# zhengjingsen/LidarDetection

Measured on AMD Instinct MI355X. Metric: frames/sec (fwd+NMS) PointPillar-KITTI, higher is better.
Workload: dtype f32; 1 GPU; PointPillar-KITTI bs=16 per GPU, fp32, eval BN folded: HIP voxelize + PFN; dense 2D backbone = first layer from the pillars (sparse implicit GEMM), stride-1 3x3 layers as Winograd F(4x4,3x3) on the fp32 MFMA, strided deblocks as one fused MFMA GEMM (all this repo's HIP), the two stride-2 3x3 layers MIOpen, stride-1 deblock + 1x1 heads hipBLASLt; exact HIP top-k + decode + batched rotated NMS; clou; replicas=1

## Files before the change

include/lidar_hip.h:

```cpp
#ifndef LIDAR_HIP_H
#define LIDAR_HIP_H

#include <stddef.h>
#include <stdint.h>

#ifdef __cplusplus
extern "C" {
#endif

#define LIDAR_OK 0
#define LIDAR_ERR_ARG (-1)
#define LIDAR_ERR_LAUNCH (-2)
#define LIDAR_ERR_WORKSPACE (-3)
#define LIDAR_ERR_UNSUPPORTED (-4)

size_t lidar_voxelize_workspace_bytes(int batch, int n_max, int max_voxels);
int lidar_voxelize_workspace_init(void *ws, size_t ws_bytes, int batch, int n_max, int max_voxels, void *stream);
int lidar_voxelize(const float *points, const int *point_offsets, int batch, int n_max, int num_features,
                   const float *range6, const float *voxel_size3, const int *grid3, int max_points,
                   int max_voxels, int compact, int algo, float *voxels, int *coords, int *num_points,
                   int *voxel_offsets, void *ws, size_t ws_bytes, void *stream);
int lidar_voxelize_hostoff(const float *points, const int *point_offsets, const int *host_offsets, int batch, int n_max,
                           int num_features, const float *range6, const float *voxel_size3, const int *grid3, int max_points,
                           int max_voxels, int compact, int algo, float *voxels, int *coords, int *num_points,
// ... 7 lines not shown
                                    void *stream);
int lidar_voxelize_error_flag(void *ws, size_t ws_bytes, int batch, int n_max, int max_voxels);

size_t lidar_voxelize_cpu_scratch_bytes(int n);
int lidar_voxelize_cpu(const float *points, int n, int num_features, const float *range6, const float *voxel_size3,
                       const int *grid3, int max_points, int max_voxels, float *voxels, int *coords_zyx, int *num_points,
                       void *scratch, size_t scratch_bytes);

int lidar_pillar_vfe(const float *voxels, const void *num_points, const void *coords, int num_voxels,
                     const int *num_voxels_dev, int max_points, int num_features, const float *weight,
                     const float *scale, const float *shift, int cout, const float *voxel_size3,
                     const float *range6, int with_distance, int coords_are_float, int num_are_float,
                     float *out, void *stream);

int lidar_mean_vfe(const float *voxels, const void *num_points, int num_voxels, int max_points,
                   int num_features, int num_are_float, float *out, void *stream);

int lidar_pillar_scatter_update(const float *pillar_features, const void *coords, int coords_are_float, int num_voxels,
                                const int *num_voxels_dev, int channels, int batch, int nx, int ny, float *canvas,
                                int *prev_cells, int *prev_count, void *stream);
size_t lidar_pillar_conv_table_workspace_bytes(int batch, int nx, int ny);
int lidar_pillar_conv_table(const void *coords, int coords_are_float, int num_voxels, const int *num_voxels_dev, int batch, int nx,
                            int ny, int k, int stride, int pad, int *nbr, void *ws, size_t ws_bytes, void *stream);
size_t lidar_pillar_scatter_workspace_bytes(int batch, int nx, int ny);
int lidar_pillar_scatter(const float *pillar_features, const void *coords, int coords_are_float, int num_voxels,
                         const int *num_voxels_dev, int channels, int batch, int nx, int ny, int channels_last,
                         float *canvas, void *ws, size_t ws_bytes, void *stream);

size_t lidar_pfn_train_workspace_bytes(int num_voxels, int num_features, int cout, int with_distance);
int lidar_pfn_train_forward(const float *voxels, const void *num_points, const void *coords, int num_voxels, const int *num_voxels_dev,
                            int max_points, int num_features, const float *weight, const float *gamma, const float *beta, int cout,
                            float eps, const float *voxel_size3, const float *range6, int with_distance, int coords_are_float,
                            int num_are_float, float *out, float *zsel, unsigned char *slot, double *stats, float *scale_shift,
                            float *batch_stats, void *ws, size_t ws_bytes, void *stream);
int lidar_pfn_train_backward(const float *voxels, const void *num_points, const void *coords, int num_voxels, const int *num_voxels_dev,
                             int max_points, int num_features, const float *weight, const float *gamma, int cout,
                             const float *voxel_size3, const float *range6, int with_distance, int coords_are_float, int num_are_float,
                             const float *grad_out, const float *zsel, const unsigned char *slot, const double *stats,
                             const float *scale_shift, float *d_weight, float *d_gamma, float *d_beta, void *ws, size_t ws_bytes,
                             void *stream);
int lidar_pillar_scatter_backward(const float *grad_canvas, const void *coords, int coords_are_float, int num_voxels,
                                  const int *num_voxels_dev, int channels, int batch, int nx, int ny, int channels_last,
                                  float *grad_features, void *stream);

size_t lidar_bn_relu_train_workspace_bytes(long long rows, int channels);
int lidar_bn_relu_train_forward(int nseg, void *const *x, const int *x_ld, const int *x_off, const int *seg_C, long long rows,
// ... 113 lines not shown
int lidar_spconv_grid_table(const int *out_indices, int n_out, int batch, int D, int H, int W, int kD, int kH, int kW, int sD, int sH, int sW,
                            int pD, int pH, int pW, const int *grid_in, int limit, int *nbr, void *stream);
int lidar_spconv_grid_table_t(const int *indices, int n, int batch, int D, int H, int W, int kD, int kH, int kW, int sD, int sH, int sW, int pD,
                              int pH, int pW, const int *grid_out, int limit, int *nbr_t, void *stream);
int lidar_spconv_grid_pad_rows(int *out_indices, const int *num_dev, int cap, void *stream);
int lidar_spconv_transpose_table(const int *nbr, int n_out, int K, int n_in, int *nbr_t, void *stream);
size_t lidar_spconv_grid_outputs_workspace_bytes(int n, int K);
int lidar_spconv_grid_outputs(const int *indices, int n, int batch, int D, int H, int W, int kD, int kH, int kW, int sD, int sH, int sW, int pD,
                              int pH, int pW, int *grid_out, int *out_indices, int *num_out, void *ws, size_t ws_bytes,
                              void *stream);
int lidar_spconv_implicit_gemm(const float *in_features, const int *nbr, int n_out, int K, int Cin, int Cout,
                               const float *weight, const float *bias, float *out_features, void *stream);
int lidar_spconv_implicit_gemm_fused(const float *in_features, const int *nbr, int n_out, int K, int Cin, int Cout,
                                     const float *weight, const float *bias, const float *residual, int relu,
                                     float *out_features, void *stream);
int lidar_spconv_row_masks(const int *nbr, int n_out, int K, int *masks, void *stream);
size_t lidar_spconv_mask_group_workspace_bytes(int n_out);
int lidar_spconv_mask_group_init(void *ws, size_t ws_bytes, void *stream);
int lidar_spconv_mask_group(const int *nbr, int n_out, int K, int *masks, int *order, void *ws, size_t ws_bytes, void *stream);
int lidar_spconv_sorted_gemm_supported(int K, int Cin, int Cout);
int lidar_spconv_implicit_gemm_sorted(const float *in_features, const int *nbr, const int *row_mask, const int *order,
                                      int n_out, int K, int Cin, int Cout, const float *weight, const float *bias,
                                      const float *residual, int relu, float *out_features, void *stream);
size_t lidar_spconv_packed_floats(int K, int Cin, int Cout);
int lidar_spconv_pack_weights(const float *weight, int K, int Cin, int Cout, float *packed, void *stream);
int lidar_spconv_implicit_gemm_sorted_packed(const float *in_features, const int *nbr, const int *row_mask, const int *order,
                                             int n_out, int K, int Cin, int Cout, const float *packed, const float *bias,
                                             const float *residual, int relu, float *out_features, void *stream);
int lidar_spconv_wgrad(const float *in_features, const float *grad_out, const int *nbr, int n_out, int K, int Cin, int Cout,
                       float *grad_weight, void *stream);
int lidar_spconv_wgrad_mfma_supported(int K, int Cin, int Cout);
size_t lidar_spconv_wgrad_workspace_bytes(int n_out, int K, int Cin, int Cout);
int lidar_spconv_wgrad_mfma(const float *in_features, const float *grad_out, const int *nbr, const int *order, int n_out, int K,
                            int Cin, int Cout, float *grad_weight, void *ws, size_t ws_bytes, void *stream);
size_t lidar_sparse_to_dense_workspace_bytes(int batch, int D, int H, int W);
int lidar_sparse_to_dense(const float *features, const int *indices, int n, int channels, int batch, int D, int H, int W,
                          float *out, void *ws, size_t ws_bytes, void *stream);

int lidar_bias_act_nhwc(const float *in, const float *bias, long long n_pix, int C, int relu, float *out, int out_C,
                        int out_off, void *stream);
int lidar_bias_act_upsample_nhwc(const float *in, const float *bias, int batch, int h, int w, int s, int C, int relu,
                                 float *out, int out_C, int out_off, void *stream);
int lidar_dense_gemm_bias_act(const float *A, long long M, int K, const float *W, int N, const float *bias, int relu,
                              float *D, int ldd, void *ws, size_t ws_bytes, void *stream);
int lidar_dense_gemm_export_choices(int *out7, int cap);
int lidar_dense_gemm_import_choices(const int *in7, int n);
// ... 198 lines not shown
```

lidardetection_amd/_lib.py:

```python
import ctypes as C
import os

_HERE = os.path.dirname(os.path.abspath(__file__))
SO_PATH = os.environ.get("LIDAR_HIP_SO") or os.path.join(_HERE, "csrc", "liblidar_hip.so")

vp, i32, f32, sz = C.c_void_p, C.c_int, C.c_float, C.c_size_t

SIGNATURES = {
    "lidar_voxelize_workspace_bytes": (sz, [i32, i32, i32]),
    "lidar_voxelize_workspace_init": (i32, [vp, sz, i32, i32, i32, vp]),
    "lidar_voxelize": (i32, [vp, vp, i32, i32, i32, vp, vp, vp, i32, i32, i32, i32, vp, vp, vp, vp, vp, sz, vp]),
    "lidar_voxelize_hostoff": (i32, [vp, vp, vp, i32, i32, i32, vp, vp, vp, i32, i32, i32, i32, vp, vp, vp, vp, vp, sz, vp]),
    "lidar_voxelize_error_flag": (i32, [vp, sz, i32, i32, i32]),
    "lidar_timer_create": (vp, []),
    "lidar_timer_destroy": (None, [vp]),
    "lidar_voxelize_time_next": (None, [vp]),
    "lidar_timer_elapsed_ms": (C.c_float, [vp]),
    "lidar_timer_parts_ms": (i32, [vp, vp]),
    "lidar_voxelize_set_error_mirror": (i32, [vp, sz, i32, i32, i32, vp, vp]),
    "lidar_pillar_vfe": (i32, [vp, vp, vp, i32, vp, i32, i32, vp, vp, vp, i32, vp, vp, i32, i32, i32, vp, vp]),
    "lidar_mean_vfe": (i32, [vp, vp, i32, i32, i32, i32, vp, vp]),
    "lidar_pillar_scatter_workspace_bytes": (sz, [i32, i32, i32]),
    "lidar_pillar_scatter": (i32, [vp, vp, i32, i32, vp, i32, i32, i32, i32, i32, vp, vp, sz, vp]),
    "lidar_pillar_scatter_update": (i32, [vp, vp, i32, i32, vp, i32, i32, i32, i32, vp, vp, vp, vp]),
    "lidar_pillar_conv_table_workspace_bytes": (sz, [i32, i32, i32]),
    "lidar_pillar_conv_table": (i32, [vp, i32, i32, vp, i32, i32, i32, i32, i32, i32, vp, vp, sz, vp]),
    "lidar_pfn_train_workspace_bytes": (sz, [i32, i32, i32, i32]),
    "lidar_pfn_train_forward": (i32, [vp, vp, vp, i32, vp, i32, i32, vp, vp, vp, i32, f32, vp, vp, i32, i32, i32, vp, vp, vp, vp, vp,
                                      vp, vp, sz, vp]),
    "lidar_pfn_train_backward": (i32, [vp, vp, vp, i32, vp, i32, i32, vp, vp, i32, vp, vp, i32, i32, i32, vp, vp, vp, vp, vp, vp, vp,
                                       vp, vp, sz, vp]),
    "lidar_pillar_scatter_backward": (i32, [vp, vp, i32, i32, vp, i32, i32, i32, i32, i32, vp, vp]),
    "lidar_bn_relu_train_workspace_bytes": (sz, [C.c_longlong, i32]),
    "lidar_bn_relu_train_forward": (i32, [i32, vp, vp, vp, vp, C.c_longlong, vp, vp, f32, vp, i32, i32, vp, vp, vp, vp, sz, vp]),
    "lidar_bn_relu_train_backward": (i32, [i32, vp, vp, vp, vp, C.c_longlong, vp, i32, i32, vp, vp, vp, vp, vp, vp, vp, sz, vp]),
    "lidar_bn_add_relu_train_forward": (i32, [vp, i32, vp, i32, i32, C.c_longlong, vp, vp, f32, vp, i32, vp, vp, vp, vp, sz, vp]),
    "lidar_bn_add_relu_train_backward": (i32, [vp, i32, vp, i32, i32, C.c_longlong, vp, i32, vp, vp, vp, vp, vp, i32, vp, vp, vp, sz, vp]),
    "lidar_iou_workspace_bytes": (sz, [i32, i32]),
    "lidar_boxes_pairwise_bev": (i32, [vp, i32, vp, i32, i32, vp, vp, sz, vp]),
    "lidar_nms_workspace_bytes": (sz, [i32, i32]),
    "lidar_nms_batch": (i32, [vp, vp, i32, i32, f32, i32, vp, vp, vp, sz, vp]),
    "lidar_nms_batch_limited": (i32, [vp, vp, i32, i32, f32, i32, i32, vp, vp, vp, sz, vp]),
    "lidar_nms_mask_ptr": (vp, [vp, i32, i32]),
    "lidar_ball_query_stack": (i32, [i32, i32, f32, i32, vp, vp, vp, vp, vp, vp]),
    "lidar_ball_query_stack2": (i32, [i32, i32, f32, i32, f32, i32, vp, vp, vp, vp, vp, vp, vp]),
    "lidar_ball_query_grid_workspace_bytes": (sz, [i32, i32]),
    "lidar_ball_query_stack_grid": (i32, [i32, i32, i32, f32, i32, f32, i32, vp, vp, vp, vp, vp, vp, vp, sz, vp]),
    "lidar_group_points_stack": (i32, [i32, i32, i32, i32, vp, vp, vp, vp, vp, vp]),
    "lidar_group_rows_stack": (i32, [i32, i32, i32, i32, i32, i32, vp, vp, vp, vp, vp, vp, vp, vp]),
# ... 27 lines not shown
    "lidar_roipoint_pool3d_forward": (i32, [i32, i32, i32, i32, i32, vp, vp, vp, vp, vp, vp]),
    "lidar_spconv_hash_capacity": (sz, [i32]),
    "lidar_spconv_build_hash": (i32, [vp, i32, i32, i32, i32, vp, sz, vp]),
    "lidar_spconv_subm_table": (i32, [vp, i32, i32, i32, i32, i32, i32, i32, vp, sz, vp, vp]),
    "lidar_spconv_conv_table_workspace_bytes": (sz, [i32, i32, i32, i32, i32, i32, i32]),
    "lidar_spconv_conv_outputs": (i32, [vp, i32, i32, i32, i32, i32, i32, i32, i32, i32, i32, i32, i32, i32, i32, vp, i32, vp, vp, sz, vp]),
    "lidar_spconv_conv_tables": (i32, [i32, i32, i32, i32, i32, i32, i32, i32, vp, vp, vp, sz, vp]),
    "lidar_spconv_grid_init": (i32, [vp, sz, vp]),
    "lidar_spconv_grid_rows": (i32, [vp, i32, vp, i32, i32, i32, i32, vp, i32, vp]),
    "lidar_spconv_grid_table": (i32, [vp, i32, i32, i32, i32, i32, i32, i32, i32, i32, i32, i32, i32, i32, i32, vp, i32, vp, vp]),
    "lidar_spconv_grid_table_t": (i32, [vp, i32, i32, i32, i32, i32, i32, i32, i32, i32, i32, i32, i32, i32, i32, vp, i32, vp, vp]),
    "lidar_spconv_grid_pad_rows": (i32, [vp, vp, i32, vp]),
    "lidar_spconv_transpose_table": (i32, [vp, i32, i32, i32, vp, vp]),
    "lidar_spconv_grid_outputs_workspace_bytes": (sz, [i32, i32]),
    "lidar_spconv_grid_outputs": (i32, [vp, i32, i32, i32, i32, i32, i32, i32, i32, i32, i32, i32, i32, i32, i32, vp, vp, vp, vp, sz, vp]),
    "lidar_spconv_implicit_gemm": (i32, [vp, vp, i32, i32, i32, i32, vp, vp, vp, vp]),
    "lidar_spconv_implicit_gemm_fused": (i32, [vp, vp, i32, i32, i32, i32, vp, vp, vp, i32, vp, vp]),
    "lidar_spconv_row_masks": (i32, [vp, i32, i32, vp, vp]),
    "lidar_spconv_mask_group_workspace_bytes": (sz, [i32]),
    "lidar_spconv_mask_group_init": (i32, [vp, sz, vp]),
    "lidar_spconv_mask_group": (i32, [vp, i32, i32, vp, vp, vp, sz, vp]),
    "lidar_spconv_sorted_gemm_supported": (i32, [i32, i32, i32]),
    "lidar_spconv_implicit_gemm_sorted": (i32, [vp, vp, vp, vp, i32, i32, i32, i32, vp, vp, vp, i32, vp, vp]),
    "lidar_spconv_packed_floats": (sz, [i32, i32, i32]),
    "lidar_spconv_pack_weights": (i32, [vp, i32, i32, i32, vp, vp]),
    "lidar_spconv_implicit_gemm_sorted_packed": (i32, [vp, vp, vp, vp, i32, i32, i32, i32, vp, vp, vp, i32, vp, vp]),
    "lidar_spconv_wgrad": (i32, [vp, vp, vp, i32, i32, i32, i32, vp, vp]),
    "lidar_spconv_wgrad_mfma_supported": (i32, [i32, i32, i32]),
    "lidar_spconv_wgrad_workspace_bytes": (sz, [i32, i32, i32, i32]),
    "lidar_spconv_wgrad_mfma": (i32, [vp, vp, vp, vp, i32, i32, i32, i32, vp, vp, sz, vp]),
    "lidar_sparse_to_dense_workspace_bytes": (sz, [i32, i32, i32, i32]),
    "lidar_sparse_to_dense": (i32, [vp, vp, i32, i32, i32, i32, i32, i32, vp, vp, sz, vp]),
    "lidar_sparse_to_bev_nhwc": (i32, [vp, vp, i32, i32, i32, i32, i32, i32, vp, vp, sz, vp]),
    "lidar_sparse_to_bev_nhwc_backward": (i32, [vp, i32, i32, vp, i32, i32, i32, i32, i32, i32, vp, vp]),
    "lidar_bias_act_nhwc": (i32, [vp, vp, C.c_longlong, i32, i32, vp, i32, i32, vp]),
    "lidar_bias_act_upsample_nhwc": (i32, [vp, vp, i32, i32, i32, i32, i32, i32, vp, i32, i32, vp]),
    "lidar_dense_gemm_bias_act": (i32, [vp, C.c_longlong, i32, vp, i32, vp, i32, vp, i32, vp, sz, vp]),
    "lidar_dense_gemm_export_choices": (i32, [vp, i32]),
    "lidar_dense_gemm_import_choices": (i32, [vp, i32]),
    "lidar_wino_packed_floats": (sz, [i32, i32]),
    "lidar_wino_supported": (i32, [i32, i32]),
    "lidar_wino_pack_weights": (i32, [vp, i32, i32, vp, vp]),
    "lidar_wino_conv3x3_nhwc": (i32, [vp, i32, i32, i32, i32, vp, vp, i32, i32, vp, i32, i32, vp]),
    "lidar_wino43_packed_floats": (sz, [i32, i32]),
    "lidar_wino43_supported": (i32, [i32, i32]),
    "lidar_wino43_pack_weights": (i32, [vp, i32, i32, vp, vp]),
# ... 183 lines not shown
```

lidardetection_amd/bev_backbone.py:

```python
import ctypes as C
import os
from typing import NamedTuple, Optional

import torch
import torch.nn as nn
import torch.nn.functional as F

from . import _lib, wino, workspace


def bias_act_(x, bias, relu=True, out=None, out_offset=0):
    _lib.require_cuda(bias)
    if not (x.is_cuda and x.dim() == 4 and x.is_contiguous(memory_format=torch.channels_last)):
        raise _lib.LidarHipError("bias_act_: expected a channels-last CUDA tensor")
    B, C, H, W = x.shape
    out, out_offset = (x, 0) if out is None else _lib.nhwc_out("bias_act_", B, (H, W), C, x.device, out, out_offset)
    _lib.check(_lib.lib().lidar_bias_act_nhwc(_lib.ptr(x), _lib.ptr(bias), B * H * W, C, int(bool(relu)), _lib.ptr(out),
                                              out.shape[1], int(out_offset), _lib.stream()), "lidar_bias_act_nhwc")
    return out


_LT_GEMM = [os.environ.get("LIDAR_BEV_LT_GEMM", "1") != "0"]
_SPLIT_MIN = [int(os.environ.get("LIDAR_BEV_SPLIT_MIN", "8"))]
_SPLIT = [int(os.environ.get("LIDAR_BEV_SPLIT", "2"))]
_WINO = [os.environ.get("LIDAR_BEV_WINO", "1") != "0"]
_DECONV = [os.environ.get("LIDAR_BEV_DECONV", "1") != "0"]
_SPARSE_FIRST = [os.environ.get("LIDAR_BEV_SPARSE_FIRST", "1") != "0"]


def _lt_gemm(a_ptr, M, K, w_kn, bias, relu, d_ptr, ldd, device):
    ws = workspace.get("dense_gemm", 32 << 20, device)
    st = _lib.lib().lidar_dense_gemm_bias_act(a_ptr, M, K, _lib.ptr(w_kn), w_kn.shape[1], _lib.ptr(bias), int(bool(relu)), d_ptr, ldd,
                                              _lib.ptr(ws), ws.numel(), _lib.stream())
    if st == -4:
        return False
    _lib.check(st, "lidar_dense_gemm_bias_act")
    return True


def _side_streams(device, n):
    from .spconv import conv as _sc, modules as _sm
    dev = torch.device(device)
    out = []
    for pool in (_sc._SIDE_STREAMS, _sm._RULEBOOK_STREAMS)[:n]:
        st = pool.get(dev)
        if st is None:
            st = pool[dev] = torch.cuda.Stream(dev, priority=-1)
        out.append(st)
    return out
# ... 198 lines not shown
        for h in heads:
            assert tuple(h.kernel_size) == (1, 1) and tuple(h.stride) == (1, 1)
        self.head_split = [h.weight.shape[0] for h in heads]
        if heads:
            self.head_wt = torch.cat([h.weight.detach().flatten(1) for h in heads], 0).t().contiguous()
            self.head_b = torch.cat([h.bias.detach() if h.bias is not None else h.weight.new_zeros(h.weight.shape[0])
                                     for h in heads], 0).contiguous()
        self._cats = {}
        self._streams = None
        self._first_sparse = None
        c0 = self.stages[0][0][0]
        w0, b0, st0, pad0 = c0.weight, c0.shift, c0.stride, c0.pad
        k0 = w0.shape[2]
        if (w0.is_cuda and w0.shape[2] == w0.shape[3] and st0[0] == st0[1] and pad0[0] == pad0[1] and k0 * k0 <= 31
                and c0.dilation == (1, 1) and c0.groups == 1 and c0.zero_pad is None):
            from .spconv import ops as _sops
            if _sops.sorted_gemm_supported(k0 * k0, w0.shape[1], w0.shape[0]):
                self._first_sparse = (w0.permute(2, 3, 1, 0).reshape(k0 * k0, w0.shape[1], w0.shape[0]).contiguous(), b0, k0, int(st0[0]), int(pad0[0]))

    def first_layer_from_pillars(self, pm):
        from . import pillar_ops
        from .spconv import ops as _sops
        w9, b0, k0, st0, pad0 = self._first_sparse
        nbr, OH, OW = pillar_ops.pillar_conv_table(pm.coords, pm.B, pm.nx, pm.ny, k0, st0, pad0, pm.num_voxels_dev)
        order = _sops.mask_order(nbr)
        out = _sops.indice_conv_fused(pm.features, nbr, w9, b0, None, True, order)
        return out.view(pm.B, OH, OW, w9.shape[2]).permute(0, 3, 1, 2)

    def sparse_first_ok(self):
        return self._first_sparse is not None and _SPARSE_FIRST[0]

    def features(self, canvas, slot=0, first_done=False):
        x, cat, off = canvas, None, 0
        for si, (convs, up) in enumerate(self.stages):
            for ci, cv in enumerate(convs):
                if first_done and si == 0 and ci == 0:
                    continue
                if cv.wino is not None and _WINO[0] and x.is_contiguous(memory_format=torch.channels_last):
                    x = wino.conv3x3_auto(x, cv.wino, cv.weight.shape[0], cv.shift, True)
                    continue
                if cv.zero_pad is not None:
                    x = F.pad(x, cv.zero_pad)
                x = _cl(F.conv2d(x, cv.weight, None, cv.stride, cv.pad, cv.dilation, cv.groups))
                bias_act_(x, cv.shift)
            B, _, h, w = x.shape
            y = None
# ... 69 lines not shown
```

lidardetection_amd/csrc/pillar.hip:

```cpp
#include "common.h"

struct PfnParams {
    float vx, vy, vz, xo, yo, zo;
    int P, C, cout, nfeat;
    int with_distance, coords_are_float, num_are_float;
};

__device__ __forceinline__ float pfn_sum32(float v) {
    v += __int_as_float(__builtin_amdgcn_update_dpp(0, __float_as_int(v), 0xB1, 0xf, 0xf, true));
    v += __int_as_float(__builtin_amdgcn_update_dpp(0, __float_as_int(v), 0x4E, 0xf, 0xf, true));
    v += __int_as_float(__builtin_amdgcn_update_dpp(0, __float_as_int(v), 0x141, 0xf, 0xf, true));
    v += __int_as_float(__builtin_amdgcn_update_dpp(0, __float_as_int(v), 0x140, 0xf, 0xf, true));
    return __int_as_float(__builtin_amdgcn_readlane(__float_as_int(v), 0)) + __int_as_float(__builtin_amdgcn_readlane(__float_as_int(v), 16));
}

template <int C, bool DIST>
__global__ __launch_bounds__(256) void pfn_kernel(const float *__restrict__ voxels, const void *__restrict__ num_points,
                                                  const void *__restrict__ coords, const float *__restrict__ weight ,
                                                  const float *__restrict__ scale, const float *__restrict__ shift,
                                                  const int *__restrict__ nvox_dev, int nvox_host, PfnParams p,
                                                  float *__restrict__ out ) {
    constexpr int NF = C + 6 + (DIST ? 1 : 0);
    const int l = lane_id();
    const int nv = nvox_dev ? min(*nvox_dev, nvox_host) : nvox_host;
// ... 426 lines not shown
}

LIDAR_EXPORT int lidar_pillar_conv_table(const void *coords, int coords_are_float, int num_voxels, const int *num_voxels_dev, int batch,
                                         int nx, int ny, int k, int stride, int pad, int *nbr, void *ws, size_t ws_bytes, void *stream) {
    if (!coords || !nbr || !ws || batch <= 0 || nx <= 0 || ny <= 0 || num_voxels < 0 || k <= 0 || k > 5 || stride <= 0 || pad < 0)
        return LIDAR_ERR_ARG;
    if (ws_bytes < lidar_pillar_conv_table_workspace_bytes(batch, nx, ny)) return LIDAR_ERR_WORKSPACE;
    const int OH = (ny + 2 * pad - k) / stride + 1, OW = (nx + 2 * pad - k) / stride + 1;
    if (OH <= 0 || OW <= 0) return LIDAR_ERR_ARG;
    const long long cells = (long long)batch * nx * ny, total = (long long)batch * OH * OW * k * k;
    if (cells > 0x7fffffffll || total > 0x7fffffffll * 256ll) return LIDAR_ERR_ARG;
    hipStream_t s = (hipStream_t)stream;
    int *map = (int *)ws;
    int fb = divup(cells, 256 * 4);
    if (fb > 2048) fb = 2048;
    hipLaunchKernelGGL(scatter_fill_kernel, dim3(fb), dim3(256), 0, s, map, cells);
    if (num_voxels > 0)
        hipLaunchKernelGGL(scatter_index_kernel, dim3(divup(num_voxels, 256)), dim3(256), 0, s, coords, coords_are_float, num_voxels,
                           num_voxels_dev, batch, nx, ny, ny, map);
    hipLaunchKernelGGL(pillar_conv_table_kernel, dim3((unsigned)divup(total, 256)), dim3(256), 0, s, map, batch, ny, nx, OH, OW, k, stride, pad, nbr);
    return lidar_check_launch("lidar_pillar_conv_table");
}

template <int CH>
__global__ __launch_bounds__(256) void canvas_clear_cells_kernel(const int *__restrict__ prev_cells, const int *__restrict__ prev_count,
                                                                 int cap, float *__restrict__ canvas) {
    constexpr int Q = CH / 4;
    const long long e = (long long)blockIdx.x * 256 + threadIdx.x;
    const int n = min(*prev_count, cap);
    const long long v = e / Q;
    if (v >= n) return;
    const int cell = prev_cells[v];
    if (cell >= 0) reinterpret_cast<float4 *>(canvas)[(long long)cell * Q + (e - v * Q)] = make_float4(0.f, 0.f, 0.f, 0.f);
}

template <int CH>
__global__ __launch_bounds__(256) void canvas_write_cells_kernel(const float *__restrict__ feat, const void *__restrict__ coords,
                                                                 int coords_are_float, int nvox_host, const int *__restrict__ nvox_dev,
                                                                 int B, int nx, int ny, float *__restrict__ canvas,
                                                                 int *__restrict__ prev_cells, int *__restrict__ prev_count) {
    constexpr int Q = CH / 4;
    const int nv = nvox_dev ? min(*nvox_dev, nvox_host) : nvox_host;
    const long long e = (long long)blockIdx.x * 256 + threadIdx.x;
    if (e == 0) *prev_count = nv;
    const long long v = e / Q;
    if (v >= nv) return;
// ... 110 lines not shown
```

lidardetection_amd/csrc/sparse_conv.hip:

```cpp
#include "common.h"
#ifndef SC_PROBE
#define SC_PROBE 0
#endif
#include <stdlib.h>

#define SC_EMPTY 0xFFFFFFFFFFFFFFFFull

struct ScGeom {
    int B, D, H, W;
    int oD, oH, oW;
    int kD, kH, kW, K;
    int sD, sH, sW, pD, pH, pW;
};

__device__ __forceinline__ unsigned long long sc_key(int b, int z, int y, int x, int D, int H, int W) {
    return (((unsigned long long)b * D + z) * H + y) * W + x;
}

__device__ __forceinline__ unsigned sc_hash(unsigned long long key, unsigned mask) {
    key ^= key >> 33;
    key *= 0xff51afd7ed558ccdull;
    key ^= key >> 33;
    return (unsigned)key & mask;
}
// ... 500 lines not shown
            const int col = q * 32 + (l & 31);
            const int cc = min(col, Cout - 1);
            const float bv = bias ? bias[cc] : 0.f;
            float res[8];
#pragma unroll
            for (int j = 0; j < 8; ++j) res[j] = 0.f;
            if (residual) {
#pragma unroll
                for (int j = 0; j < 8; ++j) res[j] = residual[(size_t)orow[j] * Cout + cc];
            }
#pragma unroll
            for (int j = 0; j < 8; ++j) {
                const int r = h * 8 + j;
                const int row = row0 + (r & 3) + 8 * (r >> 2) + 4 * (l >> 5);
                if (row < n_out && col < Cout) {
                    const float v = acc[q][r] + bv + res[j];
                    out[(size_t)orow[j] * Cout + col] = relu ? fmaxf(v, 0.f) : v;
                }
            }
        }
    }
}

template <int NT, int C4, int SL = 1>
__global__ __launch_bounds__(256) void sc_implicit_gemm_rega_kernel(const float *__restrict__ in, const int *__restrict__ nbr, int n_out,
                                                                    int K, int Cout, const float *__restrict__ Wt,
                                                                    const float *__restrict__ bias, const float *__restrict__ residual,
                                                                    int relu, float *__restrict__ out,
                                                                    const int *__restrict__ row_mask, const int *__restrict__ out_row) {
    constexpr int Cin = C4 * 4, HALF = Cin / 2, CW = NT * 32, CW4 = CW / 4, CinT = Cin * SL;
    constexpr int NG = HALF / 4;
    constexpr int NW = (Cin * CW4 + 255) / 256;
    extern __shared__ float s_mem[];
    const int t = threadIdx.x, l = t & 63, wv = t >> 6;
    const int row0 = blockIdx.x * IG_ROWS + wv * 32;
    const int ar = l & 31, ak = l >> 5;
    const int myrow = row0 + ar;
    const int trow = (out_row && myrow < n_out) ? out_row[myrow] : myrow;
    const int Co4 = Cout >> 2;
    f32x16 acc[NT];
#pragma unroll
    for (int q = 0; q < NT; ++q)
#pragma unroll
        for (int r = 0; r < 16; ++r) acc[q][r] = 0.f;
    __shared__ unsigned s_wmask[4];
    unsigned wave_mask = 0xffffffffu, wg_mask = 0xffffffffu;
    if (row_mask) {
        unsigned m = (myrow < n_out) ? (unsigned)row_mask[trow] : 0u;
#pragma unroll
        for (int d = 1; d < 64; d <<= 1) m |= (unsigned)__shfl_xor((int)m, d, 64);
        wave_mask = m;
        if (l == 0) s_wmask[wv] = m;
        __syncthreads();
        wg_mask = s_wmask[0] | s_wmask[1] | s_wmask[2] | s_wmask[3];
    }
    auto next_k = [&](int k) {
// ... 981 lines not shown
    int lg = 0;
    while (((size_t)1 << lg) < cap) ++lg;
    hipStream_t s = (hipStream_t)stream;
    hipLaunchKernelGGL(mg_insert_kernel, dim3(divup(n_out, MG_ROWS)), dim3(MG_ROWS), 0, s, nbr, n_out, K, masks, w, 32 - lg);
    hipLaunchKernelGGL(mg_assign_kernel, dim3(divup((long long)cap, 1024)), dim3(1024), 0, s, w, K, cap);
    hipLaunchKernelGGL(mg_scatter_kernel, dim3(divup(n_out > MG_BINS ? n_out : MG_BINS, 256)), dim3(256), 0, s, n_out, w, order);
    return lidar_check_launch("lidar_spconv_mask_group");
}

LIDAR_EXPORT int lidar_spconv_sorted_gemm_supported(int K, int Cin, int Cout) {
    return (K > 0 && K <= 32 && (Cout & 3) == 0 && Cout > 0 && Cout <= IG_MAX_C &&
            (Cin == 16 || Cin == 32 || Cin == 64 || Cin == 128)) ? 1 : 0;
}

LIDAR_EXPORT int lidar_spconv_implicit_gemm_sorted(const float *in_features, const int *nbr, const int *row_mask,
                                                   const int *out_row, int n_out, int K, int Cin, int Cout,
                                                   const float *weight, const float *bias, const float *residual, int relu,
                                                   float *out_features, void *stream) {
    if (!lidar_spconv_sorted_gemm_supported(K, Cin, Cout) || (n_out > 0 && (!row_mask || !out_row))) return LIDAR_ERR_ARG;
    return sc_gemm_launch(in_features, nbr, n_out, K, Cin, Cout, weight, bias, residual, relu, out_features, row_mask,
                          out_row, stream);
}

LIDAR_EXPORT size_t lidar_spconv_packed_floats(int K, int Cin, int Cout) {
    if (!sc_pk_supported(K, Cin, Cout)) return 0;
    return (size_t)K * Cin * divup(Cout, 32) * 32;
}

LIDAR_EXPORT int lidar_spconv_pack_weights(const float *weight, int K, int Cin, int Cout, float *packed, void *stream) {
    if (!weight || !packed || !sc_pk_supported(K, Cin, Cout) || (reinterpret_cast<uintptr_t>(packed) & 15)) return LIDAR_ERR_ARG;
    const long long total = (long long)lidar_spconv_packed_floats(K, Cin, Cout) / 4;
    hipLaunchKernelGGL(sc_pack_weights_kernel, dim3(divup(total, 256)), dim3(256), 0, (hipStream_t)stream, weight, K, Cin, Cout,
                       sc_pk_stage_cin(Cin), divup(Cout, 32), reinterpret_cast<float4 *>(packed), total);
    return lidar_check_launch("lidar_spconv_pack_weights");
}

LIDAR_EXPORT int lidar_spconv_implicit_gemm_sorted_packed(const float *in_features, const int *nbr, const int *row_mask,
                                                          const int *out_row, int n_out, int K, int Cin, int Cout,
                                                          const float *packed, const float *bias, const float *residual, int relu,
                                                          float *out_features, void *stream) {
    if (!lidar_spconv_sorted_gemm_supported(K, Cin, Cout) || !sc_pk_supported(K, Cin, Cout) || (n_out > 0 && (!row_mask || !out_row)) ||
        !packed || (reinterpret_cast<uintptr_t>(packed) & 15))
        return LIDAR_ERR_ARG;
    return sc_gemm_launch(in_features, nbr, n_out, K, Cin, Cout, packed, bias, residual, relu, out_features, row_mask, out_row, stream,
                          packed);
}
// ... 220 lines not shown
```

lidardetection_amd/pillar_ops.py:

```python
import torch

from . import _lib, bn_train, workspace


def fold_bn(gamma, beta, mean, var, eps):
    scale = gamma / torch.sqrt(var + eps)
    return scale.contiguous(), (beta - mean * scale).contiguous()


def pillar_vfe(voxels, num_points, coords, weight, scale, shift, voxel_size, point_cloud_range,
               with_distance=False, num_voxels_dev=None):
    _lib.require_cuda(voxels, num_points, coords, weight, scale, shift)
    V, P, C = voxels.shape
    cout = weight.shape[0]
    if weight.shape[1] != C + 6 + int(bool(with_distance)):
        raise _lib.LidarHipError("weight must be (cout, C + 6 [+1 with_distance]) — use_absolute_xyz layout")
    if coords.dtype not in (torch.int32, torch.float32) or num_points.dtype not in (torch.int32, torch.float32):
        raise _lib.LidarHipError("coords / num_points must be int32 or float32")
    out = torch.empty((V, cout), dtype=torch.float32, device=voxels.device)
    L = _lib.lib()
    _lib.check(L.lidar_pillar_vfe(_lib.ptr(voxels), _lib.ptr(num_points), _lib.ptr(coords), V, _lib.ptr(num_voxels_dev),
                                  P, C, _lib.ptr(weight), _lib.ptr(scale), _lib.ptr(shift), cout,
                                  _lib.host_f32(voxel_size), _lib.host_f32(point_cloud_range), int(bool(with_distance)),
                                  int(coords.dtype == torch.float32), int(num_points.dtype == torch.float32),
# ... 41 lines not shown
        V, C = pillar_features.shape
        if C != self.C or V > self.cap:
            raise _lib.LidarHipError("ResidentCanvas.update: feature width / pillar count exceeds what the canvas was built for")
        _lib.check(_lib.lib().lidar_pillar_scatter_update(_lib.ptr(pillar_features), _lib.ptr(coords), int(coords.dtype == torch.float32), V,
                                                          _lib.ptr(num_voxels_dev), C, self.B, self.nx, self.ny, _lib.ptr(self.canvas),
                                                          _lib.ptr(self.prev_cells), _lib.ptr(self.prev_count), _lib.stream()),
                   "lidar_pillar_scatter_update")
        return self.canvas


def pillar_conv_table(coords, batch_size, nx, ny, k, stride, pad, num_voxels_dev=None):
    _lib.require_cuda(coords)
    if coords.dtype not in (torch.int32, torch.float32) or coords.dim() != 2 or coords.shape[1] != 4:
        raise _lib.LidarHipError("pillar_conv_table: coords must be (V, 4) [b, z, y, x] int32 or float32")
    OH, OW = (ny + 2 * pad - k) // stride + 1, (nx + 2 * pad - k) // stride + 1
    L = _lib.lib()
    nbr = torch.empty((batch_size * OH * OW, k * k), dtype=torch.int32, device=coords.device)
    wsb = L.lidar_pillar_conv_table_workspace_bytes(batch_size, nx, ny)
    ws = workspace.get("pillar_conv_table", wsb, coords.device)
    _lib.check(L.lidar_pillar_conv_table(_lib.ptr(coords), int(coords.dtype == torch.float32), coords.shape[0], _lib.ptr(num_voxels_dev),
                                         batch_size, nx, ny, int(k), int(stride), int(pad), _lib.ptr(nbr), _lib.ptr(ws), wsb, _lib.stream()),
               "lidar_pillar_conv_table")
    return nbr, OH, OW


class PillarMap:

    def __init__(self, features, coords, num_voxels_dev, batch_size, nx, ny, dense_fn):
        self.features, self.coords, self.num_voxels_dev = features, coords, num_voxels_dev
        self.B, self.nx, self.ny, self._dense_fn = batch_size, nx, ny, dense_fn

    def dense(self):
        return self._dense_fn(self.features, self.coords, self.num_voxels_dev)


_STATS_DOUBLES = 272


def pfn_train_supported(num_features, max_points, cout):
    return 3 <= int(num_features) <= 8 and 0 < int(max_points) <= 64 and 0 < int(cout) <= 64


class _PillarVFETrain(torch.autograd.Function):
    @staticmethod
    def forward(ctx, meta, voxels, num_points, coords, num_voxels_dev, weight, gamma, beta):
        V, P, C = voxels.shape
# ... 103 lines not shown
```

lidardetection_amd/spconv/ops.py:

```python
import torch
from torch.autograd import Function

from .. import _lib, workspace


def get_conv_output_size(input_size, kernel_size, stride, padding, dilation=None):
    return [(i + 2 * p - k) // s + 1 for i, k, s, p in zip(input_size, kernel_size, stride, padding)]


def _hash_table(indices, spatial_shape):
    L = _lib.lib()
    n = indices.shape[0]
    cap = L.lidar_spconv_hash_capacity(n)
    table = torch.empty(cap * 12, dtype=torch.uint8, device=indices.device)
    D, H, W = spatial_shape
    _lib.check(L.lidar_spconv_build_hash(_lib.ptr(indices), n, D, H, W, _lib.ptr(table), cap, _lib.stream()), "lidar_spconv_build_hash")
    return table, cap


class GridPool:
    MAX_BYTES_PER_GRID = int(__import__("os").environ.get("LIDAR_SPCONV_GRID_MAX_GB", "8")) << 30
    MAX_TOTAL_BYTES = int(__import__("os").environ.get("LIDAR_SPCONV_GRID_TOTAL_GB", "64")) << 30
    ENABLED = __import__("os").environ.get("LIDAR_SPCONV_GRID", "1") != "0"

# ... 394 lines not shown
        return out
    if residual is not None and tuple(residual.shape) != (n_out, Cout):
        raise _lib.LidarHipError("indice_conv_fused: residual must be (n_out, Cout)")
    if order is not None and packed is not None and PACKED_GEMM[0]:
        masks, perm = order
        _lib.check(_lib.lib().lidar_spconv_implicit_gemm_sorted_packed(_lib.ptr(feats), _lib.ptr(nbr), _lib.ptr(masks), _lib.ptr(perm),
                                                                       n_out, K, Cin, Cout, _lib.ptr(packed), _lib.ptr(bias),
                                                                       _lib.ptr(residual), int(bool(relu)), _lib.ptr(out), _lib.stream()),
                   "lidar_spconv_implicit_gemm_sorted_packed")
        return out
    if order is not None:
        masks, perm = order
        _lib.check(_lib.lib().lidar_spconv_implicit_gemm_sorted(_lib.ptr(feats), _lib.ptr(nbr), _lib.ptr(masks), _lib.ptr(perm),
                                                                n_out, K, Cin, Cout, _lib.ptr(weight_kcc), _lib.ptr(bias),
                                                                _lib.ptr(residual), int(bool(relu)), _lib.ptr(out), _lib.stream()),
                   "lidar_spconv_implicit_gemm_sorted")
        return out
    _lib.check(_lib.lib().lidar_spconv_implicit_gemm_fused(_lib.ptr(feats), _lib.ptr(nbr), n_out, K, Cin, Cout,
                                                           _lib.ptr(weight_kcc), _lib.ptr(bias), _lib.ptr(residual), int(bool(relu)),
                                                           _lib.ptr(out), _lib.stream()), "lidar_spconv_implicit_gemm_fused")
    return out


class SparseConvFunction(Function):

    @staticmethod
    def forward(ctx, features, weight, bias, fwd_table, bwd_table, flip_bwd, orders=None):
        feats = features.contiguous()
        Cin, Cout = weight.shape[-2], weight.shape[-1]
        w = weight.reshape(-1, Cin, Cout).contiguous()
        _lib.require_cuda(feats, w, fwd_table)
        order = None
        if orders is not None and fwd_table.shape[0] > 0 and sorted_gemm_supported(w.shape[0], Cin, Cout):
            order = cached_mask_order(orders[0], orders[1], fwd_table)
        out = _implicit_gemm(feats, fwd_table, w, bias.contiguous() if bias is not None else None, fwd_table.shape[0], order)
        ctx.save_for_backward(feats, w, fwd_table, bwd_table)
        ctx.flip_bwd, ctx.has_bias, ctx.wshape, ctx.orders = flip_bwd, bias is not None, weight.shape, orders
        return out

    @staticmethod
    def backward(ctx, grad_out):
        feats, w, fwd_table, bwd_table = ctx.saved_tensors
        g = grad_out.contiguous()
        K, Cin, Cout = w.shape
        grad_feats = grad_w = grad_b = None
        if ctx.needs_input_grad[0]:
# ... 29 lines not shown
```

Measured before the change: 3302 frames/s.

## Fuse first-layer neighbor table and mask ordering, skip empty-row tiles in GEMM

```diff
diff --git a/include/lidar_hip.h b/include/lidar_hip.h
--- a/include/lidar_hip.h
+++ b/include/lidar_hip.h
@@ -53,6 +53,11 @@
 size_t lidar_pillar_conv_table_workspace_bytes(int batch, int nx, int ny);
 int lidar_pillar_conv_table(const void *coords, int coords_are_float, int num_voxels, const int *num_voxels_dev, int batch, int nx,
                             int ny, int k, int stride, int pad, int *nbr, void *ws, size_t ws_bytes, void *stream);
+int lidar_pillar_first_layer_supported(int k, int stride, int pad);
+size_t lidar_pillar_first_layer_workspace_bytes(int batch, int nx, int ny, int k, int stride, int pad);
+int lidar_pillar_first_layer_order(const void *coords, int coords_are_float, int num_voxels, const int *num_voxels_dev, int batch,
+                                   int nx, int ny, int k, int stride, int pad, int *nbr, int *masks, int *order, int *tail_start,
+                                   void *ws, size_t ws_bytes, void *stream);
 size_t lidar_pillar_scatter_workspace_bytes(int batch, int nx, int ny);
 int lidar_pillar_scatter(const float *pillar_features, const void *coords, int coords_are_float, int num_voxels,
                          const int *num_voxels_dev, int channels, int batch, int nx, int ny, int channels_last,
@@ -212,6 +217,10 @@
 int lidar_spconv_implicit_gemm_sorted(const float *in_features, const int *nbr, const int *row_mask, const int *order,
                                       int n_out, int K, int Cin, int Cout, const float *weight, const float *bias,
                                       const float *residual, int relu, float *out_features, void *stream);
+int lidar_spconv_sorted_tail_gemm_supported(int K, int Cin, int Cout);
+int lidar_spconv_implicit_gemm_sorted_tail(const float *in_features, const int *nbr, const int *row_mask, const int *order,
+                                           const int *tail_start, int n_out, int K, int Cin, int Cout, const float *weight,
+                                           const float *bias, int relu, float *out_features, void *stream);
 size_t lidar_spconv_packed_floats(int K, int Cin, int Cout);
 int lidar_spconv_pack_weights(const float *weight, int K, int Cin, int Cout, float *packed, void *stream);
 int lidar_spconv_implicit_gemm_sorted_packed(const float *in_features, const int *nbr, const int *row_mask, const int *order,
diff --git a/lidardetection_amd/_lib.py b/lidardetection_amd/_lib.py
--- a/lidardetection_amd/_lib.py
+++ b/lidardetection_amd/_lib.py
@@ -25,6 +25,9 @@
     "lidar_pillar_scatter_update": (i32, [vp, vp, i32, i32, vp, i32, i32, i32, i32, vp, vp, vp, vp]),
     "lidar_pillar_conv_table_workspace_bytes": (sz, [i32, i32, i32]),
     "lidar_pillar_conv_table": (i32, [vp, i32, i32, vp, i32, i32, i32, i32, i32, i32, vp, vp, sz, vp]),
+    "lidar_pillar_first_layer_supported": (i32, [i32, i32, i32]),
+    "lidar_pillar_first_layer_workspace_bytes": (sz, [i32, i32, i32, i32, i32, i32]),
+    "lidar_pillar_first_layer_order": (i32, [vp, i32, i32, vp, i32, i32, i32, i32, i32, i32, vp, vp, vp, vp, vp, sz, vp]),
     "lidar_pfn_train_workspace_bytes": (sz, [i32, i32, i32, i32]),
     "lidar_pfn_train_forward": (i32, [vp, vp, vp, i32, vp, i32, i32, vp, vp, vp, i32, f32, vp, vp, i32, i32, i32, vp, vp, vp, vp, vp,
                                       vp, vp, sz, vp]),
@@ -98,6 +101,8 @@
     "lidar_spconv_mask_group": (i32, [vp, i32, i32, vp, vp, vp, sz, vp]),
     "lidar_spconv_sorted_gemm_supported": (i32, [i32, i32, i32]),
     "lidar_spconv_implicit_gemm_sorted": (i32, [vp, vp, vp, vp, i32, i32, i32, i32, vp, vp, vp, i32, vp, vp]),
+    "lidar_spconv_sorted_tail_gemm_supported": (i32, [i32, i32, i32]),
+    "lidar_spconv_implicit_gemm_sorted_tail": (i32, [vp, vp, vp, vp, vp, i32, i32, i32, i32, vp, vp, i32, vp, vp]),
     "lidar_spconv_packed_floats": (sz, [i32, i32, i32]),
     "lidar_spconv_pack_weights": (i32, [vp, i32, i32, i32, vp, vp]),
     "lidar_spconv_implicit_gemm_sorted_packed": (i32, [vp, vp, vp, vp, i32, i32, i32, i32, vp, vp, vp, i32, vp, vp]),
diff --git a/lidardetection_amd/bev_backbone.py b/lidardetection_amd/bev_backbone.py
--- a/lidardetection_amd/bev_backbone.py
+++ b/lidardetection_amd/bev_backbone.py
@@ -25,6 +25,7 @@
 _SPLIT = [int(os.environ.get("LIDAR_BEV_SPLIT", "2"))]
 _WINO = [os.environ.get("LIDAR_BEV_WINO", "1") != "0"]
 _DECONV = [os.environ.get("LIDAR_BEV_DECONV", "1") != "0"]
+_FIRST_ORDER = [os.environ.get("LIDAR_BEV_FIRST_ORDER", "1") != "0"]
 _SPARSE_FIRST = [os.environ.get("LIDAR_BEV_SPARSE_FIRST", "1") != "0"]
 
 
@@ -269,6 +270,11 @@
         from . import pillar_ops
         from .spconv import ops as _sops
         w9, b0, k0, st0, pad0 = self._first_sparse
+        if (_FIRST_ORDER[0] and pillar_ops.first_layer_order_supported(k0, st0, pad0) and _sops.sorted_tail_gemm_supported(*w9.shape)
+                and b0.data_ptr() % 16 == 0):
+            nbr, order, tail, OH, OW = pillar_ops.pillar_first_layer_order(pm.coords, pm.B, pm.nx, pm.ny, k0, st0, pad0, pm.num_voxels_dev)
+            out = _sops.indice_conv_sorted_tail(pm.features, nbr, w9, b0, True, order, tail)
+            return out.view(pm.B, OH, OW, w9.shape[2]).permute(0, 3, 1, 2)
         nbr, OH, OW = pillar_ops.pillar_conv_table(pm.coords, pm.B, pm.nx, pm.ny, k0, st0, pad0, pm.num_voxels_dev)
         order = _sops.mask_order(nbr)
         out = _sops.indice_conv_fused(pm.features, nbr, w9, b0, None, True, order)
diff --git a/lidardetection_amd/csrc/pillar.hip b/lidardetection_amd/csrc/pillar.hip
--- a/lidardetection_amd/csrc/pillar.hip
+++ b/lidardetection_amd/csrc/pillar.hip
@@ -472,6 +472,204 @@
     return lidar_check_launch("lidar_pillar_conv_table");
 }
 
+#define PFL_ROWS 1024
+#define PFL_MAXK 9
+#define PFL_MAXBINS (1 << PFL_MAXK)
+
+__global__ void pfl_fill_kernel(int *__restrict__ map, long long n, int *__restrict__ totals, int nbins) {
+    const long long n4 = n >> 2;
+    const long long tid = (long long)blockIdx.x * blockDim.x + threadIdx.x;
+    const long long stride = (long long)gridDim.x * blockDim.x;
+    for (long long i = tid; i < n4; i += stride) reinterpret_cast<int4 *>(map)[i] = make_int4(-1, -1, -1, -1);
+    if (tid < (n & 3)) map[(n4 << 2) + tid] = -1;
+    if (tid < nbins) totals[tid] = 0;
+}
+
+__global__ __launch_bounds__(PFL_ROWS) void pfl_table_kernel(const int *__restrict__ map, int ny, int nx, int OH, int OW, int k, int stride,
+                                                             int pad, int n, int *__restrict__ nbr, int *__restrict__ masks,
+                                                             int *__restrict__ rank, int *__restrict__ wghist, int *__restrict__ totals,
+                                                             int vec_ok) {
+    const int nwg = gridDim.x;
+    __shared__ __align__(16) int s_nbr[PFL_ROWS * PFL_MAXK];
+    __shared__ unsigned short s_wcnt[PFL_ROWS / 64][PFL_MAXBINS];
+    const int t = threadIdx.x, l = t & 63, wv = t >> 6;
+    const int K = k * k, nbins = 1 << K;
+    const int row0 = blockIdx.x * PFL_ROWS, row = row0 + t;
+    const bool valid = row < n;
+    unsigned m = 0u;
+    if (valid) {
+        const int ox = row % OW, o = row / OW;
+        const int oy = o % OH, b = o / OH;
+        const int *mb = map + (size_t)b * ny * nx;
+        const int iy0 = oy * stride - pad, ix0 = ox * stride - pad;
+#pragma unroll
+        for (int ky = 0; ky < 3; ++ky) {
+#pragma unroll
+            for (int kx = 0; kx < 3; ++kx) {
+                if (ky < k && kx < k) {
+                    const int iy = iy0 + ky, ix = ix0 + kx, tap = ky * k + kx;
+                    const int v = (iy >= 0 && iy < ny && ix >= 0 && ix < nx) ? mb[(size_t)iy * nx + ix] : -1;
+                    s_nbr[t * K + tap] = v;
+                    if (v >= 0) m |= 1u << tap;
+                }
+            }
+        }
+        masks[row] = (int)m;
+    }
+    for (int i = t; i < (PFL_ROWS / 64) * PFL_MAXBINS / 2; i += PFL_ROWS) reinterpret_cast<unsigned *>(&s_wcnt[0][0])[i] = 0u;
+    __syncthreads();
+    int lrank = 0;
+    unsigned long long todo = __ballot(valid);
+    while (todo) {
+        const int leader = __ffsll((long long)todo) - 1;
+        const unsigned m0 = (unsigned)__shfl((int)m, leader, 64);
+        const unsigned long long same = __ballot(valid && m == m0);
+        if (valid && m == m0) lrank = __popcll(same & ((1ull << l) - 1ull));
+        if (l == leader) s_wcnt[wv][m0] = (unsigned short)__popcll(same);
+        todo &= ~same;
+    }
+    __syncthreads();
+    if (t < nbins) {
+        int run = 0;
+#pragma unroll
+        for (int w = 0; w < PFL_ROWS / 64; ++w) {
+            const int c = s_wcnt[w][t];
+            s_wcnt[w][t] = (unsigned short)run;
+            run += c;
+        }
+        wghist[(size_t)t * nwg + blockIdx.x] = run;
+        if (run) atomicAdd(&totals[t], run);
+    }
+    __syncthreads();
+    if (valid) rank[row] = (int)s_wcnt[wv][m] + lrank;
+    const int cnt = min(PFL_ROWS, n - row0) * K;
+    int *dst = nbr + (size_t)row0 * K;
+    int done = 0;
+    if (vec_ok) {
+        const int cnt4 = cnt >> 2;
+        for (int i = t; i < cnt4; i += PFL_ROWS) reinterpret_cast<int4 *>(dst)[i] = reinterpret_cast<const int4 *>(s_nbr)[i];
+        done = cnt4 << 2;
+    }
+    for (int i = done + t; i < cnt; i += PFL_ROWS) dst[i] = s_nbr[i];
+}
+
+__device__ __forceinline__ bool pfl_before(int a, int b) {
+    const int pa = __popc((unsigned)a), pb = __popc((unsigned)b);
+    return pa > pb || (pa == pb && a < b);
+}
+
+__device__ __forceinline__ int pfl_block_excl_scan(int v, int *s_w, int *total) {
+    const int t = threadIdx.x, l = t & 63, wv = t >> 6;
+    const int inc = wave_incl_scan(v);
+    __syncthreads();
+    if (l == 63) s_w[wv] = inc;
+    __syncthreads();
+    int o = inc - v;
+    for (int w = 0; w < wv; ++w) o += s_w[w];
+    *total = s_w[0] + s_w[1] + s_w[2] + s_w[3];
+    return o;
+}
+
+__global__ __launch_bounds__(256) void pfl_scan_kernel(const int *__restrict__ totals, int nbins, int nwg, int *__restrict__ wghist,
+                                                       int *__restrict__ tail_start) {
+    __shared__ int s_w[4];
+    constexpr int PER = 8;
+    const int t = threadIdx.x, bin = blockIdx.x;
+    int base = 0;
+    for (int g0 = 0; g0 < nwg; g0 += 256 * PER) {
+        const int g1 = min(g0 + 256 * PER, nwg), per = (g1 - g0 + 255) / 256;
+        const int w0 = min(g0 + t * per, g1), w1 = min(w0 + per, g1);
+        int c[PER], mine = 0;
+#pragma unroll
+        for (int j = 0; j < PER; ++j) {
+            c[j] = (w0 + j < w1) ? wghist[(size_t)bin * nwg + w0 + j] : 0;
+            mine += c[j];
+        }
+        if (g0 == 0) {
+            const int own = totals[bin];
+            int before = 0;
+            for (int q = t; q < nbins; q += 256)
+                if (pfl_before(q, bin)) before += totals[q];
+            if (own == 0 && bin != 0) return;
+            pfl_block_excl_scan(before, s_w, &base);
+            if (bin == 0 && t == 0) *tail_start = base;
+        }
+        int total;
+        int run = base + pfl_block_excl_scan(mine, s_w, &total);
+#pragma unroll
+        for (int j = 0; j < PER; ++j) {
+            if (w0 + j < w1) wghist[(size_t)bin * nwg + w0 + j] = run;
+            run += c[j];
+        }
+        base += total;
+    }
+}
+
+__global__ void pfl_scatter_kernel(const int *__restrict__ masks, const int *__restrict__ rank, const int *__restrict__ wghist, int nwg,
+                                   int n, int *__restrict__ order) {
+    const int r = blockIdx.x * blockDim.x + threadIdx.x;
+    if (r < n) order[wghist[(size_t)masks[r] * nwg + r / PFL_ROWS] + rank[r]] = r;
+}
+
+LIDAR_EXPORT int lidar_pillar_first_layer_supported(int k, int stride, int pad) {
+    return (k > 0 && k * k <= PFL_MAXK && stride > 0 && pad >= 0) ? 1 : 0;
+}
+
+struct PflGeom {
+    int OH, OW, K, nbins, nwg;
+    long long cells, n;
+    size_t off_map, off_rank, off_hist, bytes;
+};
+
+static bool pfl_geom(int batch, int nx, int ny, int k, int stride, int pad, PflGeom *g) {
+    if (!lidar_pillar_first_layer_supported(k, stride, pad) || batch <= 0 || nx <= 0 || ny <= 0) return false;
+    g->OH = (ny + 2 * pad - k) / stride + 1;
+    g->OW = (nx + 2 * pad - k) / stride + 1;
+    if (ny + 2 * pad < k || nx + 2 * pad < k || g->OH <= 0 || g->OW <= 0) return false;
+    g->K = k * k;
+    g->nbins = 1 << g->K;
+    g->cells = (long long)batch * nx * ny;
+    g->n = (long long)batch * g->OH * g->OW;
+    if (g->cells > 0x7fffffffll || g->n * g->K > 0x7fffffffll) return false;
+    g->nwg = divup(g->n, PFL_ROWS);
+    g->off_map = align_up((size_t)PFL_MAXBINS * 4, 256);
+    g->off_rank = g->off_map + align_up((size_t)g->cells * 4, 256);
+    g->off_hist = g->off_rank + align_up((size_t)g->n * 4, 256);
+    g->bytes = g->off_hist + align_up((size_t)g->nwg * g->nbins * 4, 256);
+    return true;
+}
+
+LIDAR_EXPORT size_t lidar_pillar_first_layer_workspace_bytes(int batch, int nx, int ny, int k, int stride, int pad) {
+    PflGeom g;
+    return pfl_geom(batch, nx, ny, k, stride, pad, &g) ? g.bytes : 0;
+}
+
+LIDAR_EXPORT int lidar_pillar_first_layer_order(const void *coords, int coords_are_float, int num_voxels, const int *num_voxels_dev,
+                                                int batch, int nx, int ny, int k, int stride, int pad, int *nbr, int *masks, int *order,
+                                                int *tail_start, void *ws, size_t ws_bytes, void *stream) {
+    PflGeom g;
+    if (!coords || !nbr || !masks || !order || !tail_start || !ws || num_voxels < 0 || !pfl_geom(batch, nx, ny, k, stride, pad, &g))
+        return LIDAR_ERR_ARG;
+    if ((reinterpret_cast<uintptr_t>(ws) & 15) || (reinterpret_cast<uintptr_t>(nbr) & 3)) return LIDAR_ERR_ARG;
+    if (ws_bytes < g.bytes) return LIDAR_ERR_WORKSPACE;
+    hipStream_t s = (hipStream_t)stream;
+    int *totals = (int *)ws, *map = (int *)((char *)ws + g.off_map), *rank = (int *)((char *)ws + g.off_rank);
+    int *wghist = (int *)((char *)ws + g.off_hist);
+    const int n = (int)g.n;
+    int fb = divup(g.cells, 256 * 4);
+    if (fb > 2048) fb = 2048;
+    if (fb < divup(g.nbins, 256)) fb = divup(g.nbins, 256);
+    hipLaunchKernelGGL(pfl_fill_kernel, dim3(fb), dim3(256), 0, s, map, g.cells, totals, g.nbins);
+    if (num_voxels > 0)
+        hipLaunchKernelGGL(scatter_index_kernel, dim3(divup(num_voxels, 256)), dim3(256), 0, s, coords, coords_are_float, num_voxels,
+                           num_voxels_dev, batch, nx, ny, ny, map);
+    hipLaunchKernelGGL(pfl_table_kernel, dim3(g.nwg), dim3(PFL_ROWS), 0, s, map, ny, nx, g.OH, g.OW, k, stride, pad, n, nbr, masks, rank,
+                       wghist, totals, (int)((reinterpret_cast<uintptr_t>(nbr) & 15) == 0));
+    hipLaunchKernelGGL(pfl_scan_kernel, dim3(g.nbins), dim3(256), 0, s, totals, g.nbins, g.nwg, wghist, tail_start);
+    hipLaunchKernelGGL(pfl_scatter_kernel, dim3(divup(n, 256)), dim3(256), 0, s, masks, rank, wghist, g.nwg, n, order);
+    return lidar_check_launch("lidar_pillar_first_layer_order");
+}
+
 template <int CH>
 __global__ __launch_bounds__(256) void canvas_clear_cells_kernel(const int *__restrict__ prev_cells, const int *__restrict__ prev_count,
                                                                  int cap, float *__restrict__ canvas) {
diff --git a/lidardetection_amd/csrc/sparse_conv.hip b/lidardetection_amd/csrc/sparse_conv.hip
--- a/lidardetection_amd/csrc/sparse_conv.hip
+++ b/lidardetection_amd/csrc/sparse_conv.hip
@@ -546,16 +546,32 @@
     }
 }
 
-template <int NT, int C4, int SL = 1>
+template <int NT, int C4, int SL = 1, bool TAIL = false>
 __global__ __launch_bounds__(256) void sc_implicit_gemm_rega_kernel(const float *__restrict__ in, const int *__restrict__ nbr, int n_out,
                                                                     int K, int Cout, const float *__restrict__ Wt,
                                                                     const float *__restrict__ bias, const float *__restrict__ residual,
                                                                     int relu, float *__restrict__ out,
-                                                                    const int *__restrict__ row_mask, const int *__restrict__ out_row) {
+                                                                    const int *__restrict__ row_mask, const int *__restrict__ out_row,
+                                                                    const int *__restrict__ tail_start = nullptr) {
     constexpr int Cin = C4 * 4, HALF = Cin / 2, CW = NT * 32, CW4 = CW / 4, CinT = Cin * SL;
     constexpr int NG = HALF / 4;
     constexpr int NW = (Cin * CW4 + 255) / 256;
     extern __shared__ float s_mem[];
+    if constexpr (TAIL) {
+        const int tile0 = blockIdx.x * IG_ROWS;
+        if (tile0 >= *tail_start) {
+            const int C4o = Cout >> 2;
+            for (int e = threadIdx.x; e < IG_ROWS * C4o; e += 256) {
+                const int r = e / C4o, q4 = e - r * C4o;
+                if (tile0 + r >= n_out) break;
+                float4 v = bias ? reinterpret_cast<const float4 *>(bias)[q4] : make_float4(0.f, 0.f, 0.f, 0.f);
+                v.x = 0.f + v.x + 0.f; v.y = 0.f + v.y + 0.f; v.z = 0.f + v.z + 0.f; v.w = 0.f + v.w + 0.f;
+                if (relu) { v.x = fmaxf(v.x, 0.f); v.y = fmaxf(v.y, 0.f); v.z = fmaxf(v.z, 0.f); v.w = fmaxf(v.w, 0.f); }
+                reinterpret_cast<float4 *>(out)[(size_t)out_row[tile0 + r] * C4o + q4] = v;
+            }
+            return;
+        }
+    }
     const int t = threadIdx.x, l = t & 63, wv = t >> 6;
     const int row0 = blockIdx.x * IG_ROWS + wv * 32;
     const int ar = l & 31, ak = l >> 5;
@@ -1583,6 +1599,25 @@
                           out_row, stream);
 }
 
+LIDAR_EXPORT int lidar_spconv_sorted_tail_gemm_supported(int K, int Cin, int Cout) {
+    return (lidar_spconv_sorted_gemm_supported(K, Cin, Cout) && Cin == 64) ? 1 : 0;
+}
+
+LIDAR_EXPORT int lidar_spconv_implicit_gemm_sorted_tail(const float *in_features, const int *nbr, const int *row_mask, const int *out_row,
+                                                        const int *tail_start, int n_out, int K, int Cin, int Cout, const float *weight,
+                                                        const float *bias, int relu, float *out_features, void *stream) {
+    if (!lidar_spconv_sorted_tail_gemm_supported(K, Cin, Cout) || n_out < 0) return LIDAR_ERR_ARG;
+    if (n_out == 0) return LIDAR_OK;
+    if (!in_features || !nbr || !row_mask || !out_row || !tail_start || !weight || !out_features) return LIDAR_ERR_ARG;
+    if ((reinterpret_cast<uintptr_t>(bias) & 15) || (reinterpret_cast<uintptr_t>(out_features) & 15)) return LIDAR_ERR_ARG;
+    const dim3 grid(divup(n_out, IG_ROWS));
+    const size_t lds = (size_t)2 * 64 * divup(Cout, 32) * 32 * sizeof(float);
+#define IGT(NT) hipLaunchKernelGGL((sc_implicit_gemm_rega_kernel<NT, 16, 1, true>), grid, dim3(256), lds, (hipStream_t)stream, in_features, nbr, n_out, K, Cout, weight, bias, nullptr, relu, out_features, row_mask, out_row, tail_start)
+    switch (divup(Cout, 32)) { case 1: IGT(1); break; case 2: IGT(2); break; case 3: IGT(3); break; default: IGT(4); break; }
+#undef IGT
+    return lidar_check_launch("lidar_spconv_implicit_gemm_sorted_tail");
+}
+
 LIDAR_EXPORT size_t lidar_spconv_packed_floats(int K, int Cin, int Cout) {
     if (!sc_pk_supported(K, Cin, Cout)) return 0;
     return (size_t)K * Cin * divup(Cout, 32) * 32;
diff --git a/lidardetection_amd/pillar_ops.py b/lidardetection_amd/pillar_ops.py
--- a/lidardetection_amd/pillar_ops.py
+++ b/lidardetection_amd/pillar_ops.py
@@ -87,6 +87,31 @@
                                          batch_size, nx, ny, int(k), int(stride), int(pad), _lib.ptr(nbr), _lib.ptr(ws), wsb, _lib.stream()),
                "lidar_pillar_conv_table")
     return nbr, OH, OW
+
+
+def first_layer_order_supported(k, stride, pad):
+    return bool(_lib.lib().lidar_pillar_first_layer_supported(int(k), int(stride), int(pad)))
+
+
+def pillar_first_layer_order(coords, batch_size, nx, ny, k, stride, pad, num_voxels_dev=None):
+    _lib.require_cuda(coords)
+    if coords.dtype not in (torch.int32, torch.float32) or coords.dim() != 2 or coords.shape[1] != 4:
+        raise _lib.LidarHipError("pillar_first_layer_order: coords must be (V, 4) [b, z, y, x] int32 or float32")
+    L = _lib.lib()
+    wsb = L.lidar_pillar_first_layer_workspace_bytes(batch_size, nx, ny, int(k), int(stride), int(pad))
+    if wsb == 0:
+        raise _lib.LidarHipError("pillar_first_layer_order: this map / kernel is not supported (first_layer_order_supported)")
+    OH, OW = (ny + 2 * pad - k) // stride + 1, (nx + 2 * pad - k) // stride + 1
+    n = batch_size * OH * OW
+    nbr = torch.empty((n, k * k), dtype=torch.int32, device=coords.device)
+    aux = torch.empty(2 * n + 4, dtype=torch.int32, device=coords.device)
+    masks, order, tail = aux[:n], aux[n:2 * n], aux[2 * n:2 * n + 1]
+    ws = workspace.get("pillar_first_layer_order", wsb, coords.device)
+    _lib.check(L.lidar_pillar_first_layer_order(_lib.ptr(coords), int(coords.dtype == torch.float32), coords.shape[0], _lib.ptr(num_voxels_dev),
+                                                batch_size, nx, ny, int(k), int(stride), int(pad), _lib.ptr(nbr), _lib.ptr(masks),
+                                                _lib.ptr(order), _lib.ptr(tail), _lib.ptr(ws), wsb, _lib.stream()),
+               "lidar_pillar_first_layer_order")
+    return nbr, (masks, order), tail, OH, OW
 
 
 class PillarMap:
diff --git a/lidardetection_amd/spconv/ops.py b/lidardetection_amd/spconv/ops.py
--- a/lidardetection_amd/spconv/ops.py
+++ b/lidardetection_amd/spconv/ops.py
@@ -440,6 +440,25 @@
     return out
 
 
+def sorted_tail_gemm_supported(K, Cin, Cout):
+    return bool(_lib.lib().lidar_spconv_sorted_tail_gemm_supported(K, Cin, Cout))
+
+
+def indice_conv_sorted_tail(feats, nbr, weight_kcc, bias, relu, order, tail_start):
+    K, Cin, Cout = weight_kcc.shape
+    n_out = nbr.shape[0]
+    _lib.require_cuda(feats, weight_kcc, nbr, bias, tail_start)
+    out = torch.empty((n_out, Cout), dtype=torch.float32, device=feats.device)
+    if n_out == 0:
+        return out
+    masks, perm = order
+    _lib.check(_lib.lib().lidar_spconv_implicit_gemm_sorted_tail(_lib.ptr(feats), _lib.ptr(nbr), _lib.ptr(masks), _lib.ptr(perm),
+                                                                 _lib.ptr(tail_start), n_out, K, Cin, Cout, _lib.ptr(weight_kcc),
+                                                                 _lib.ptr(bias), int(bool(relu)), _lib.ptr(out), _lib.stream()),
+               "lidar_spconv_implicit_gemm_sorted_tail")
+    return out
+
+
 class SparseConvFunction(Function):
 
     @staticmethod
```

After: 3334 frames/s, median of 6. About the same (+1.0%).
